# benoriol/hand_pose_sl

Hardware: NVIDIA B200
Metric: body2hand_train_frames_per_sec (higher is better)
Workload: dtype bf16

## Files before the change

hand_pose_sl_b200/csrc/b2h_capi.cu:

```cuda
#include <atomic>
#include <cstdarg>
#include <cstdio>
#include <mutex>
#include <cmath>

#include "b2h_common.cuh"

namespace b2h {

static thread_local char g_err[512] = "";
static std::atomic<long long> g_launches{0};

void set_error(const char* fmt, ...) {
  va_list ap;
  va_start(ap, fmt);
  vsnprintf(g_err, sizeof(g_err), fmt, ap);
  va_end(ap);
}
int check_launch(const char* what) {
  cudaError_t e = cudaGetLastError();
  if (e != cudaSuccess) {
    set_error("%s: %s", what, cudaGetErrorString(e));
    return B2H_ECUDA;
  }
// ... 231 lines not shown
  if ((reinterpret_cast<uintptr_t>(x) & 15) || (reinterpret_cast<uintptr_t>(target) & talign) ||
      (reinterpret_cast<uintptr_t>(conf) & calign) || (reinterpret_cast<uintptr_t>(packed) & 15)) {
    if (wv) set_error("%s: frames and packed must be 16-byte aligned, target_frames 8-byte and conf_frames 4-byte aligned", who);
    else set_error("%s: x, target and packed must be 16-byte aligned", who);
    return B2H_EALIGN;
  }
  g = make_geo(n_in, C, pos_emb);
  plan = train_plan(g, B, T, precision);
  if (wv && plan.kernel != B2H_KERNEL_TC_TILE && plan.kernel != B2H_KERNEL_TC_WIDE_TRAIN) {
    set_error("%s: window views are trained on the tensor cores: in bf16 mode for conv_channels <= 32 with at most 32 input "
              "channels and T <= 4096, and for conv_channels <= 256 with T <= 256; in fp32 mode for conv_channels <= 32 with at "
              "most 32 input channels and T <= 4096; materialise the windows (b2h_preprocess) for C=%d, T=%d, precision=%d",
              who, C, T, precision);
    return B2H_ESHAPE;
  }
  if (plan.kernel == B2H_KERNEL_NONE) {
    set_error("%s: no training kernel for conv_channels=%d, T=%d, precision=%d (tcgen05 training: C <= 32 in the one-launch tile "
              "kernel, C <= 256 in bf16 mode through the wide kernels, T <= 256; the FFMA kernel would need %zu B of shared memory)",
              who, C, T, precision, plan.ffma.smem);
    return B2H_ESHAPE;
  }
  const int nparts = plan.nparts;
  const int64_t stride = plan.stride;
  if (workspace_bytes < plan.total - 256) { set_error("%s: workspace %lld B < %lld B", who, (long long)workspace_bytes, (long long)plan.total); return B2H_EWORKSPACE; }
  if (reinterpret_cast<uintptr_t>(workspace) & 15) { set_error("%s: workspace must be 16-byte aligned", who); return B2H_EALIGN; }
  partials = reinterpret_cast<float*>(reinterpret_cast<char*>(workspace) + B2H_WS_HEADER);
  loss_partials = partials + (size_t)nparts * stride;
  Fp32Args a{};
  a.x = x; a.x_dtype = x_dtype; a.target = target; a.conf = conf; a.d_y = d_y; a.lengths = lengths; a.params = params;
  a.packed = reinterpret_cast<const char*>(packed); a.y = pred_out; a.partials = partials; a.loss_partials = loss_partials;
  a.B = B; a.T = T; a.loss_kind = loss_kind; a.apply_mask = 1; a.mode = mode; a.out_scale = 1.0f; a.geo = g;
  a.step_dev = step_dev;
  a.epoch_dev = epoch_dev;
  if (wv) a.wv = *wv;
  if (plan.kernel == B2H_KERNEL_TC_TILE) {
    if (fuse) {
      if (nparts > B2H_WS_MAX_CTA) { set_error("%s: %d CTAs exceed the %d arrival flags of the workspace header", who, nparts, B2H_WS_MAX_CTA); return B2H_ESHAPE; }
      fuse->enabled = 1;
      fuse->hdr = reinterpret_cast<unsigned*>(workspace);
      a.fuse = *fuse;
    }
    return launch_tc_tile_train(a, plan.tile, stream);
  }
  if (plan.kernel == B2H_KERNEL_TC_WIDE_TRAIN) {
    return launch_tc_wide_train(a, plan.wide, reinterpret_cast<unsigned char*>(workspace) + plan.scratch_off, stream);
  }
  return launch_fp32(a, plan.ffma, stream);
}

static int train_forward_backward(const void* x, int x_dtype, const WindowView* wv, const float* target, const float* conf,
                                  const int32_t* lengths, const float* params, const void* packed, float* grads_out,
                                  float* loss_out, float* pred_out, int B, int T, int n_in, int C, int pos_emb, int loss_kind,
                                  int precision, int64_t* step_dev, void* workspace, int64_t workspace_bytes, void* stream,
                                  const char* who) {
  if (grads_out && !loss_out) { set_error("%s: null loss_out", who); return B2H_EINVAL; }
  Geo g; TrainPlan plan; float *partials, *loss_partials;
  int rc = train_common(x, x_dtype, wv, target, conf, nullptr, lengths, params, packed, pred_out, B, T, n_in, C, pos_emb,
                        loss_kind, precision, 1, workspace, workspace_bytes, (cudaStream_t)stream, g, plan, partials,
                        loss_partials, who, reinterpret_cast<long long*>(step_dev));
  if (rc || !grads_out) return rc;
  return launch_reduce(partials, plan.nparts, plan.gp_layout, g, grads_out, loss_partials, loss_out, (cudaStream_t)stream, nullptr, plan.n_loss);
}

extern "C" int b2h_train_forward_backward(const void* x, int x_dtype, const float* target, const float* conf,
                                          const int32_t* lengths, const float* params, const void* packed,
                                          float* grads_out, float* loss_out, float* pred_out, int B, int T, int n_in,
// ... 228 lines not shown
```

hand_pose_sl_b200/csrc/b2h_common.cuh:

```cuda
#pragma once
#include <cuda_runtime.h>
#include <cuda_bf16.h>
#include <stdint.h>
#include "../../include/b2h.h"

#define B2H_KW 5
#define B2H_PADW 2
#define B2H_COUT 42
#define B2H_MAX_C 256

namespace b2h {

__host__ __device__ inline int round_up(int x, int m) { return (x + m - 1) / m * m; }

struct Geo {
  int n_in, C, pos_emb;
  int pe_len;
  int cin[4], cout[4];
  int w_off[4], b_off[4];
  int P;
  int64_t wf_off[4];
  int64_t wd_off[4];
  int64_t tf_off[4];
  int64_t td_off[4];
// ... 125 lines not shown
  const float denom = sqrtf(v) * inv_bc2_sqrt + eps;
  return p - step_size * (m / denom);
}

__host__ __device__ inline double ipow(double b, long long t) {
  double r = 1.0;
  while (t > 0) {
    if (t & 1) r *= b;
    b *= b;
    t >>= 1;
  }
  return r;
}

struct SubWindow { int start, clo, chi; };
__host__ __device__ inline int sub_window_cut(int T, int Ts, int n_sub, int i) {
  if (i <= 0) return 0;
  if (i >= n_sub) return T;
  const int c = (Ts - 16) + (i - 1) * (Ts - 32);
  return c < T ? c : T;
}
__host__ __device__ inline SubWindow sub_window(int T, int Ts, int n_sub, int i) {
  SubWindow s;
  const int cb0 = sub_window_cut(T, Ts, n_sub, i), cb1 = sub_window_cut(T, Ts, n_sub, i + 1);
  int st = cb0 - 16;
  st = st < 0 ? 0 : st;
  st = st > T - Ts ? T - Ts : st;
  s.start = st; s.clo = cb0 - st; s.chi = cb1 - st;
  return s;
}

#define B2H_WS_HEADER 1024
#define B2H_WS_MAX_CTA 192

struct FuseAdam {
  int enabled;
  float* params; float* m; float* v; char* packed;
  double lr, beta1, beta2;
  const double* lr_dev;
  float eps, grad_scale;
  const long long* step_dev;
  float* loss_out;
  unsigned* hdr;
  const float* const* peer_bufs;
  float* sym_grads;
  unsigned long long* mc_buf;
  const long long* epoch_dev;
  int rank, world;
};

void set_error(const char* fmt, ...);
int check_launch(const char* what);
void count_launch(int n = 1);


struct WindowView { const long long* win_start; const long long* win_end; long long n_frames; int pad_mode; };

__device__ __forceinline__ long long window_src_row(const WindowView& v, int w, int t) {
  const long long start = v.win_start[w];
  long long cend = v.win_end ? v.win_end[w] : v.n_frames;
  cend = cend > v.n_frames ? v.n_frames : cend;
  long long f = start + t;
  if (f >= cend || f < 0) f = (v.pad_mode == B2H_PAD_REPEAT_FIRST && start >= 0 && start < cend) ? start : -1;
  return f;
}

// ... 14 lines not shown
  size_t smem;
  int grid;
};
RowspacePlan plan_rowspace(const Geo& g, int B, int T);

struct WidePlan {
  bool ok;
  int gh, n_tiles, a_bytes, nstage;
  size_t smem;
  int grid;
  int ksplit;
  int n_loss;
  int64_t scratch_bytes;
};
WidePlan plan_wide(const Geo& g, int B, int T);

struct FfmaPlan {
  bool ok, train;
  size_t smem;
  int grid;
};
FfmaPlan plan_ffma(const Geo& g, int B, int T, bool train);

struct Fp32Args {
  const void* x; int x_dtype;
  const float* target; const float* conf; const float* d_y; const int32_t* lengths;
  const float* params; const char* packed;
  float* y;
  float* partials;
  float* loss_partials;
  long long* step_dev;
  long long* epoch_dev;
  FuseAdam fuse;
  int B, T, loss_kind, apply_mask, mode;
  float out_scale;
  Geo geo;
  WindowView wv;
};
int launch_fp32(Fp32Args& p, const FfmaPlan& plan, cudaStream_t stream);

struct TcFwdArgs {
  const void* x; int x_dtype;
  const float* params; const char* packed; const int32_t* lengths;
  float* y;
  int B, T, G, NT, RBUF, apply_mask;
  float out_scale;
  Geo geo;
  WindowView wv;
};
int launch_tc_fwd(TcFwdArgs& p, const RowspacePlan& plan, cudaStream_t stream);
int launch_tc_wide_train(const Fp32Args& a, const WidePlan& plan, unsigned char* scratch, cudaStream_t stream);
int launch_tc_wide_fwd(const void* x, int x_dtype, const float* params, const char* packed, const int32_t* lengths, float* y,
                       int B, int T, int apply_mask, float out_scale, const Geo& g, const WidePlan& plan, cudaStream_t stream,
                       const WindowView* wv);
int launch_tc_probe(const void* a, const void* b, float* out, int n, int ksteps, int shift, int variant, cudaStream_t stream);
int tc_status_and_clear();

int launch_tc_tile_fwd(const void* x, int x_dtype, const float* params, const char* packed, const int32_t* lengths, float* y,
                       int apply_mask, float out_scale, const Geo& g, const TilePlan& plan, cudaStream_t stream, const WindowView* wv);
int launch_tc_tile_train(const Fp32Args& a, const TilePlan& plan, cudaStream_t stream);

void set_debug_timing(long long* p);
int launch_tc_bench(long long* out, int M, int N, int reps, int nacc, int mn_major, cudaStream_t stream);
int launch_format_prediction(const float* pred, float* out, int64_t rows, int mode, cudaStream_t stream);
int launch_pos_emb_concat(const float* inp, float* out, int B, int Cc, int T, int max_len, cudaStream_t stream);
int launch_pack(const float* params, void* packed, const Geo& g, cudaStream_t stream);
// ... 17 lines not shown
```

hand_pose_sl_b200/csrc/b2h_conv_fp32.cu:

```cuda
#include "b2h_common.cuh"

namespace b2h {

constexpr int kThreads = 256;
constexpr int kWarps = kThreads / 32;



template <int EPI>
__device__ __forceinline__ void conv_rows(const float* __restrict__ in, int ldi, int Cin, const float* __restrict__ W,
                                          int Cout, const float* __restrict__ bias, float* __restrict__ out, int ldo,
                                          const float* __restrict__ act, int lda, int T) {
  const int lane = threadIdx.x & 31, warp = threadIdx.x >> 5;
  const int nRB = (T + 7) >> 3, nCG = (Cout + 31) >> 5;
  for (int task = warp; task < nRB * nCG; task += kWarps) {
    const int rb = task / nCG, cg = task - rb * nCG;
    const int co = cg * 32 + lane;
    const bool active = co < Cout;
    const int r0 = rb * 8;
    float acc[8];
    const float b0 = (EPI != 2 && active) ? __ldg(bias + co) : 0.0f;
#pragma unroll
    for (int j = 0; j < 8; ++j) acc[j] = b0;
    const float* xin = in + r0 * ldi;
// ... 75 lines not shown
  for (int w = 0; w < kWarps; ++w) s += red[w];
  return s;
}

template <bool TRAIN>
__global__ void __launch_bounds__(kThreads) conv_fp32_kernel(Fp32Args p) {
  extern __shared__ __align__(16) float smem[];
  __shared__ float red[kWarps];
  const Geo& g = p.geo;
  const int T = p.T;
  const int TR = round_up(T, 8) + 4;
  const int ld0 = round_up(g.cin[0], 4), ldc = round_up(g.C, 4), ldg = round_up(g.C > B2H_COUT ? g.C : B2H_COUT, 4);
  float* X = smem;
  float* A1 = X + TR * ld0;
  float* A2 = A1 + TR * ldc;
  float* A3 = A2 + TR * ldc;
  float* G0 = A3 + TR * ldc;
  float* G1 = G0 + TR * ldg;
  const int total = TRAIN ? TR * (ld0 + 3 * ldc + 2 * ldg) : TR * (ld0 + 2 * ldc);
  for (int i = threadIdx.x; i < total; i += kThreads) smem[i] = 0.0f;
  __syncthreads();

  const float* Wf[4];
  const float* Wd[4];
  const float* bias[4];
#pragma unroll
  for (int l = 0; l < 4; ++l) {
    Wf[l] = reinterpret_cast<const float*>(p.packed + g.wf_off[l]);
    Wd[l] = reinterpret_cast<const float*>(p.packed + g.wd_off[l]);
    bias[l] = p.params + g.b_off[l];
  }
  if (TRAIN && p.step_dev && blockIdx.x == 0 && threadIdx.x == 0) *p.step_dev += 1;
  if (TRAIN && p.epoch_dev && blockIdx.x == 0 && threadIdx.x == 0) *p.epoch_dev += 1;
  float* part = TRAIN ? p.partials + (size_t)blockIdx.x * g.P : nullptr;
  float loss_acc = 0.0f;
  bool first = true;

  for (int b = blockIdx.x; b < p.B; b += gridDim.x) {
    const int n_in = g.n_in, pe = g.pos_emb;
    if (p.x_dtype == B2H_DT_F32) {
      const float* xs = reinterpret_cast<const float*>(p.x) + (size_t)b * T * n_in;
      for (int i = threadIdx.x; i < T * n_in; i += kThreads) {
        int t = i / n_in, c = i - t * n_in;
        X[(t + 2) * ld0 + pe + c] = __ldg(xs + i);
      }
    } else {
      const __nv_bfloat16* xs = reinterpret_cast<const __nv_bfloat16*>(p.x) + (size_t)b * T * n_in;
      for (int i = threadIdx.x; i < T * n_in; i += kThreads) {
        int t = i / n_in, c = i - t * n_in;
        X[(t + 2) * ld0 + pe + c] = __bfloat162float(xs[i]);
      }
    }
    if (pe) {
      for (int t = threadIdx.x; t < T; t += kThreads) X[(t + 2) * ld0] = __fdiv_rn((float)t, (float)g.pe_len);
    }
    __syncthreads();
    conv_rows<0>(X, ld0, g.cin[0], Wf[0], g.cout[0], bias[0], A1, ldc, nullptr, 0, T);
    __syncthreads();
    conv_rows<0>(A1, ldc, g.cin[1], Wf[1], g.cout[1], bias[1], A2, ldc, nullptr, 0, T);
    __syncthreads();
    int len = T;
    if (p.lengths) { len = p.lengths[b]; len = len < 0 ? 0 : (len > T ? T : len); }

    if (!TRAIN) {
      conv_rows<0>(A2, ldc, g.cin[2], Wf[2], g.cout[2], bias[2], A1, ldc, nullptr, 0, T);
      __syncthreads();
// ... 138 lines not shown
```

hand_pose_sl_b200/csrc/b2h_train_tc.cuh:

```cuda
#pragma once
#include <type_traits>

namespace b2h {
using namespace tc;

struct TcTileArgs {
  const void* x; int x_dtype;
  const float* target; const float* conf; const float* d_y; const int32_t* lengths;
  const float* params; const char* packed;
  float* y;
  float* partials;
  float* loss_partials;
  long long* step_dev;
  long long* epoch_dev;
  long long* dbg;
  FuseAdam fuse;
  const long long* win_start; const long long* win_end; long long n_frames; int pad_mode;
  int T_orig, n_sub, loss_B;
  int B, T, loss_kind, apply_mask, mode;
  float out_scale;
  int n_tiles, nhalf, MB, HR, gh, NT;
  Geo geo;
};

constexpr int kTileThreads = 256;
constexpr int kAccCol = 0;
constexpr int kWgPairCols = 5 * 32 + 8;
constexpr int kGatherDepth = 24;
constexpr uint32_t kDpSentinel = 0xFFFFFFFFu;

struct TileSmem {
  int g0, g1, x, a1, a2, a3, ones, lo_off, ys, has_ys, wf[4], wlo_off, wd[4], total;
};

__host__ __device__ inline TileSmem tile_smem_layout(const Geo& g, int rows, bool train, bool split = false) {
  TileSmem s;
  const int CH = rows * 16;
  int o = 0;
  s.g0 = o; o += train ? 6 * CH : 0;
  s.g1 = o; o += train ? 4 * CH : 0;
  s.x = o;  o += (g.kp[0] / 8) * CH;
  s.a1 = o; o += (g.kp[1] / 8) * CH;
  s.a2 = o; o += (g.kp[1] / 8) * CH;
  s.a3 = o; o += train ? (g.kp[1] / 8) * CH : 0;
  s.ones = o; o += train ? CH : 0;
  s.lo_off = split ? o : 0;
  if (split) o *= 2;
// ... 57 lines not shown
      const uint32_t a = a_lo + 2 * s * rows + k, b = b_lo + (k * KS + s) * 2 * N;
      umma_bf16(d_tmem, desc64(a, a_hi), desc64(b, b_hi), idesc, acc);
      acc = 1;
      if (SPLIT) {
        umma_bf16(d_tmem, desc64(a + al16, a_hi), desc64(b, b_hi), idesc, 1);
        umma_bf16(d_tmem, desc64(a, a_hi), desc64(b + bl16, b_hi), idesc, 1);
      }
    }
  }
}

__device__ __forceinline__ void grid_barrier_flags(unsigned* hdr, unsigned tok, int tid) {
  __syncthreads();
  volatile unsigned* flags = hdr + 4;
  if (tid == 0) {
    __threadfence();
    flags[blockIdx.x] = tok;
  }
  if (tid < 32) {
    const long long t0 = clock64();
    for (;;) {
      bool mine = true;
      for (int c = tid; c < (int)gridDim.x; c += 32) mine = mine && (flags[c] == tok);
      if (__all_sync(0xffffffffu, mine)) break;
      if (clock64() - t0 > 4000000000LL) {
        if (tid == 0) atomicExch(&g_tc_status, 50);
        break;
      }
    }
    __threadfence();
  }
  __syncthreads();
}

__device__ __forceinline__ void adam_apply(const FuseAdam& f, const Geo& g, const GpSlot& slot, int i, float gr, float m, float v,
                                           float p, float step_size, float inv_bc2_sqrt) {
  p = adam_update(m, v, p, gr * f.grad_scale, (float)(1.0 - f.beta1), (float)(1.0 - f.beta2), (float)f.beta2, f.eps, step_size,
                  inv_bc2_sqrt);
  f.m[i] = m; f.v[i] = v; f.params[i] = p;
  if (f.packed) scatter_packed(g, f.packed, slot, p);
}

#define B2H_STAMP() do { if (p.dbg && blockIdx.x == 0 && tid == 0 && dbg_n < 120) p.dbg[dbg_n++] = clock64(); } while (0)
__device__ __forceinline__ long long global_ns() { long long t; asm volatile("mov.u64 %0, %globaltimer;" : "=l"(t)); return t; }
#define B2H_MARK(i) do { if (p.dbg && tid == 0 && blockIdx.x < 192) p.dbg[128 + 4 * blockIdx.x + (i)] = global_ns(); } while (0)

template <bool TRAIN, int NT, bool SPLIT, bool VIEW = false>
__global__ void __launch_bounds__(kTileThreads, 1) conv_tc_tile_kernel(TcTileArgs p) {
  int dbg_n = 0;
  extern __shared__ __align__(128) unsigned char smem[];
  __shared__ __align__(8) uint64_t bar;
  __shared__ __align__(8) uint64_t wbar;
  __shared__ __align__(8) uint64_t tbar;
  __shared__ uint32_t tmem_slot;
  __shared__ __align__(16) float bias_s[4][64];
  __shared__ float red_s[8];
  const Geo& g = p.geo;
  const int T = p.T, MB = p.MB, HR = p.HR, nhalf = p.nhalf, gh = p.gh;
  constexpr int kWgCol = 64 * NT;
  const int tid = threadIdx.x, lane = tid & 31;
  const int warp = __shfl_sync(0xffffffffu, tid >> 5, 0);
  const int rows = nhalf * HR;
  const int CH = rows * 16;
  const TileSmem L = tile_smem_layout(g, rows, TRAIN, SPLIT);
  const int LO = L.lo_off;
  const uint32_t al16 = (uint32_t)L.lo_off >> 4, bl16 = (uint32_t)L.wlo_off >> 4;
// ... 97 lines not shown
    mbar_init(&bar, nissue);
    mbar_init(&wbar, 1);
    mbar_init(&tbar, 1);
    fence_barrier_init();
  }
  auto zero_buffers = [&]() {
    const int act_bytes = L.ys;
    uint4* z = reinterpret_cast<uint4*>(smem);
    const uint4 zero = make_uint4(0, 0, 0, 0);
    for (int i = tid; i < act_bytes / 16; i += kTileThreads) z[i] = zero;
  };
  if (!TRAIN) zero_buffers();
  griddep_wait();
  B2H_STAMP();
  prefetch_x(blockIdx.x);
  if (tid == 0) {
    uint32_t total = 4 * 64 * 4;
    for (int l = 0; l < 4; ++l) {
      total += B2H_KW * g.kp[l] * g.np_[l] * 2 * (SPLIT ? 2 : 1);
      if (TRAIN && !SPLIT && l > 0) total += B2H_KW * round_up(g.cout[l], 16) * round_up(g.cin[l], 16) * 2;
    }
    mbar_arrive_expect_tx(&wbar, total);
    bulk_g2s(&bias_s[0][0], p.packed + g.bias_off, 4 * 64 * 4, &wbar);
    for (int l = 0; l < 4; ++l) {
      bulk_g2s(smem + L.wf[l], p.packed + g.tf_off[l], B2H_KW * g.kp[l] * g.np_[l] * 2, &wbar);
      if (SPLIT) bulk_g2s(smem + L.wf[l] + L.wlo_off, p.packed + g.tfl_off[l], B2H_KW * g.kp[l] * g.np_[l] * 2, &wbar);
      if (TRAIN && !SPLIT && l > 0)
        bulk_g2s(smem + L.wd[l], p.packed + g.td_off[l], B2H_KW * round_up(g.cout[l], 16) * round_up(g.cin[l], 16) * 2, &wbar);
    }
  }
  long long step_next = 0, epoch_next = 0;
  unsigned sync_tok = 0;
  int abort_flag = 0;
  if (TRAIN) {
    if (p.fuse.enabled) {
      step_next = *reinterpret_cast<const volatile long long*>(p.fuse.step_dev) + 1;
      if (p.fuse.world > 1) {
        epoch_next = *reinterpret_cast<const volatile long long*>(p.fuse.epoch_dev) + 1;
        abort_flag = *reinterpret_cast<volatile int*>(&g_dp_abort);
      }
      sync_tok = *reinterpret_cast<const volatile unsigned*>(p.fuse.hdr) + 1u;
    } else if (blockIdx.x == 0 && tid == 0) {
      if (p.step_dev) *p.step_dev += 1;
      if (p.epoch_dev) *p.epoch_dev += 1;
    }
  }
  if (TRAIN) zero_buffers();
  tc_fence_before();
  __syncthreads();
  tc_fence_after();
  const uint32_t tbase = tmem_slot;
  uint32_t phase = 0, tphase = 0;
  float loss_acc = 0.0f;
  bool wg_started = false, weights_ready = false;
  B2H_STAMP();

  const uint32_t hi_k = desc_hi(128);
  const uint32_t hi_mn = desc_hi((uint32_t)CH);
  const uint32_t acc_d = tbase + kAccCol;

  bool pair1_done = false;
  auto readout_pair = [&](int pr) {
    float* part = p.partials + (size_t)blockIdx.x * gp_total(g);
    const int l = 2 * pr + (lane >> 4);
    const int co = (warp & 3) * 16 + (lane & 15);
    const bool mine = co < g.cout[l];
    const int Nw = g.kp[l];
    float* lp = part + gp_layer_off(g, l);
    float4* lp4 = reinterpret_cast<float4*>(lp);
    const int q4 = Nw >> 2, cout_l = g.cout[l];
    const uint32_t dcol = tbase + lane_addr + kWgCol + pr * kWgPairCols;
    const int k0 = ch == 0 ? 0 : 3, nk = ch == 0 ? 3 : 2;
    uint32_t v[3][32];
#pragma unroll
    for (int k = 0; k < 3; ++k)
      if (k < nk) tmem_ld32(dcol + (k0 + k) * 32, v[k]);
    uint32_t vb[16];
    if (ch == 1) tmem_ld16(dcol + 5 * 32, vb);
    tmem_ld_wait();
    if (mine) {
#pragma unroll
      for (int k = 0; k < 3; ++k) {
        if (k >= nk) continue;
        float4* dst = lp4 + (size_t)(k0 + k) * q4 * cout_l + co;
#pragma unroll
        for (int q = 0; q < 8; ++q)
          if (q * 4 < Nw)
            dst[(size_t)q * cout_l] = make_float4(__uint_as_float(v[k][4 * q]), __uint_as_float(v[k][4 * q + 1]),
                                                  __uint_as_float(v[k][4 * q + 2]), __uint_as_float(v[k][4 * q + 3]));
      }
      if (ch == 1) lp[B2H_KW * g.cout[l] * Nw + co] = __uint_as_float(vb[0]);
    }
  };

  for (int tile = blockIdx.x; tile < p.n_tiles; tile += gridDim.x) {
    const int wbase = tile * wpt;
    int lens[NT];
#pragma unroll
    for (int j = 0; j < NT; ++j) {
      const RowCtx rc = rowctx(j, wbase);
      const int Tw = p.n_sub > 1 ? p.T_orig : T;
      lens[j] = Tw;
      if (rc.valid && p.lengths) { const int v = p.lengths[p.n_sub > 1 ? rc.gw / p.n_sub : rc.gw]; lens[j] = v < 0 ? 0 : (v > Tw ? Tw : v); }
    }

    const bool tgt_smem = TRAIN && p.mode == 1 && bulk_io && p.n_sub <= 1;
    if (tid == 0) {
      if (!TRAIN) bulk_wait_read0();
      if (tgt_smem) {
        int nw = p.B - wbase; nw = nw > wpt ? wpt : nw;
        fence_proxy_async_smem();
        if (!VIEW) {
          mbar_arrive_expect_tx(&tbar, (uint32_t)nw * T * B2H_COUT * 4);
          for (int w = 0; w < nw; ++w) {
            const int h = w / gh, j = w - h * gh;
            bulk_g2s(YS + (size_t)(h * MB + j * (T + 2)) * B2H_COUT, p.target + (size_t)(wbase + w) * T * B2H_COUT,
                     (uint32_t)T * B2H_COUT * 4, &tbar);
          }
        } else {
          int nb = 0;
          for (int w = 0; w < nw; ++w) nb += view_bulk(wbase + w) ? 1 : 0;
          mbar_arrive_expect_tx(&tbar, (uint32_t)nb * T * B2H_COUT * 4);
          for (int w = 0; w < nw; ++w) {
            if (!view_bulk(wbase + w)) continue;
            const int h = w / gh, j = w - h * gh;
// ... 57 lines not shown
        float2* dst = reinterpret_cast<float2*>(YS + (size_t)srow * B2H_COUT);
        for (int q = ch * 11; q < (ch ? B2H_COUT / 2 : 11); ++q) dst[q] = tr < 0 ? make_float2(0.f, 0.f) : __ldg(src + q);
      }
      if (TRAIN && ch == 0) {
        uint4 o = make_uint4(0, 0, 0, 0);
        if (rc.valid) o.x = 0x00003F80u;
        *reinterpret_cast<uint4*>(ONES + (size_t)row * 16) = o;
      }
    }
    prefetch_x(tile + gridDim.x);
    fence_proxy_async_smem();
    tc_fence_before();
    __syncthreads();
    tc_fence_after();
    B2H_STAMP();
    if (!weights_ready) { mbar_wait(&wbar, 0, 19); weights_ready = true; }
    B2H_STAMP();

    for (int l = 0; l < 4; ++l) {
      unsigned char* bin = (l == 0) ? X : (l == 1) ? A1 : (l == 2) ? A2 : (TRAIN ? A3 : A1);
      unsigned char* bout = (l == 0) ? A1 : (l == 1) ? A2 : (TRAIN ? A3 : A1);
      const int KS = g.kp[l] >> 4, N = g.np_[l];
      if (warp < nissue) {
        if (elect_one()) {
          const uint32_t idesc = make_idesc_bf16(idesc_M, N, 0, 0);
          const uint32_t a_lo = desc_lo(smem_u32(bin), (uint32_t)CH) + warp * seg_row;
          const uint32_t b_lo = desc_lo(smem_u32(smem + L.wf[l]), (uint32_t)N * 16);
          issue_conv<SPLIT>(acc_d + warp * seg_d, a_lo, hi_k, b_lo, hi_k, KS, N, rows, idesc, al16, bl16);
          umma_commit(&bar);
        }
        __syncwarp();
      }
      B2H_STAMP();
      mbar_wait(&bar, phase, 20 + l);
      phase ^= 1;
      tc_fence_after();
      B2H_STAMP();
      float contrib = 0.f;
#pragma unroll
      for (int j = 0; j < NT; ++j) {
      const RowCtx rc = rowctx(j, wbase);
      const int row = rc.row, t = rc.t, gw = rc.gw;
      const bool valid = rc.valid;
      const uint32_t taddr = tbase + lane_addr + kAccCol + 64 * j;
      if (l < 3) {
        for (int c0 = 16 * ch; c0 < N; c0 += 32) {
          uint32_t v[16];
          tmem_ld16(taddr + c0, v);
          tmem_ld_wait();
          float f[16];
#pragma unroll
          for (int q = 0; q < 16; ++q) f[q] = valid ? fmaxf(__uint_as_float(v[q]) + bias_s[l][c0 + q], 0.0f) : 0.0f;
          store8_act<SPLIT>(bout, LO, CH, row, c0 >> 3, f);
          store8_act<SPLIT>(bout, LO, CH, row, (c0 >> 3) + 1, f + 8);
        }
      } else {
        int len = lens[j];
        float n_el = 0.f, scale = 0.f;
        const float* tg = nullptr; const float* cf = nullptr; const float* dy = nullptr;
        const size_t drow = valid ? (size_t)dense_row(gw, t) : 0;
        bool in_core = true, zrow = false;
        if (TRAIN && valid) {
          n_el = (float)len * (float)B2H_COUT;
          scale = (p.loss_kind == B2H_LOSS_L1) ? (1.0f / (float)p.loss_B) / n_el : 1.0f / n_el;
          if (p.n_sub > 1) {
            const SubW sw = subw(gw);
// ... 212 lines not shown
          const int row = rc.row;
          const bool valid = rc.valid;
          const uint32_t taddr = tbase + lane_addr + kAccCol + 64 * j;
          for (int c0 = 16 * ch; c0 < Nd; c0 += 32) {
            uint32_t v[16];
            tmem_ld16(taddr + c0, v);
            tmem_ld_wait();
            float f[16], act[16];
            bf16x8_to_float(*reinterpret_cast<const uint4*>(ain + (size_t)(c0 >> 3) * CH + (size_t)row * 16), act);
            bf16x8_to_float(*reinterpret_cast<const uint4*>(ain + (size_t)((c0 >> 3) + 1) * CH + (size_t)row * 16), act + 8);
#pragma unroll
            for (int q = 0; q < 16; ++q) f[q] = (valid && act[q] > 0.0f) ? __uint_as_float(v[q]) : 0.0f;
            store8_act<SPLIT>(gnext, LO, CH, row, c0 >> 3, f);
            store8_act<SPLIT>(gnext, LO, CH, row, (c0 >> 3) + 1, f + 8);
          }
          }
        }
        if (l == 1 && tile + (int)gridDim.x >= p.n_tiles) {
          readout_pair(1);
          pair1_done = true;
        }
        fence_proxy_async_smem();
        tc_fence_before();
        __syncthreads();
        tc_fence_after();
        B2H_STAMP();
      }
      wg_started = true;
    }
  }

  if (TRAIN) {
    if (!wg_started) {
      float* part = p.partials + (size_t)blockIdx.x * gp_total(g);
      for (int i = tid; i < gp_total(g); i += kTileThreads) part[i] = 0.0f;
    } else {
      readout_pair(0);
      if (!pair1_done) readout_pair(1);
    }
    if (tid == 0 && p.loss_partials)
      p.loss_partials[blockIdx.x] = (p.loss_kind == B2H_LOSS_L1) ? loss_acc / (float)p.loss_B : loss_acc;
    B2H_STAMP();

    if (p.fuse.enabled) {
      const FuseAdam& f = p.fuse;
      __shared__ float s_step_size, s_inv_bc2_sqrt;
      const int nj = gp_total(g);
      const int nparts = (int)gridDim.x;
      const int per = round_up((nj + nparts - 1) / nparts, 4);
      const int j0 = (int)blockIdx.x * per;
      const int j_end = min(nj, j0 + per);
      const bool dp = f.world > 1;
      if (tid == kTileThreads - 1) {
        const float lr = (float)(f.lr_dev ? *f.lr_dev : f.lr);
        const float tt = (float)step_next;
        const float bc1 = -expm1f(tt * log1pf((float)(f.beta1 - 1.0)));
        const float bc2 = -expm1f(tt * log1pf((float)(f.beta2 - 1.0)));
        s_step_size = lr / bc1;
        s_inv_bc2_sqrt = 1.0f / sqrtf(bc2);
      }
      const bool one_pass = per <= kTileThreads;
      GpSlot my_slot;
      int my_i = -1;
      float my_m = 0.f, my_v = 0.f, my_p = 0.f;
      if (one_pass && j0 + tid < j_end && gp_decode(g, j0 + tid, my_slot)) {
        my_i = gp_flat_of_slot(g, my_slot);
        my_m = __ldcg(f.m + my_i); my_v = __ldcg(f.v + my_i); my_p = __ldcg(f.params + my_i);
      }
      B2H_MARK(1);
      bool aborted = abort_flag != 0;
      grid_barrier_flags(f.hdr, sync_tok, tid);
      B2H_STAMP();
      B2H_MARK(2);
      if (blockIdx.x == 0 && tid == 0) {
        *reinterpret_cast<volatile unsigned*>(f.hdr) = sync_tok;
        *p.step_dev = step_next;
        if (dp) *p.epoch_dev = epoch_next;
      }
      if (blockIdx.x == 0 && warp == 7 && f.loss_out) {
        float sl = 0.f;
        for (int c = lane; c < (int)gridDim.x; c += 32) sl += __ldcg(p.loss_partials + c);
#pragma unroll
        for (int o = 16; o > 0; o >>= 1) sl += __shfl_xor_sync(0xffffffffu, sl, o);
        if (lane == 0) *f.loss_out = sl;
      }
      const long long epoch = epoch_next;
      const size_t ll_src = ((size_t)(epoch & 1) * f.world + f.rank) * nj;
      float4* red4 = reinterpret_cast<float4*>(L.has_ys ? smem + L.ys : smem);
      for (int jb = j0; jb < j_end; jb += 4096) {
        const int jn = min(j_end, jb + 4096);
        const int ncol = (jn - jb + 3) >> 2;
        int groups = kTileThreads / ncol; groups = groups < 1 ? 1 : (groups > 8 ? 8 : groups);
        const int cpg = kTileThreads / groups;
        for (int cb = 0; cb < ncol; cb += cpg) {
          const int col = cb + tid % cpg, pg = tid / cpg;
          if (col < ncol && pg < groups) {
            const float4* src = reinterpret_cast<const float4*>(p.partials + jb + 4 * col);
            const size_t stride4 = (size_t)nj >> 2;
            float4 acc = make_float4(0.f, 0.f, 0.f, 0.f);
            for (int c = pg; c < nparts; c += kGatherDepth * groups) {
              float4 v[kGatherDepth];
#pragma unroll
              for (int u = 0; u < kGatherDepth; ++u) {
                const int cc = c + u * groups;
                v[u] = (cc < nparts) ? __ldcg(src + (size_t)cc * stride4) : make_float4(0.f, 0.f, 0.f, 0.f);
              }
#pragma unroll
              for (int u = 0; u < kGatherDepth; ++u) { acc.x += v[u].x; acc.y += v[u].y; acc.z += v[u].z; acc.w += v[u].w; }
            }
            red4[pg * ncol + col] = acc;
          }
        }
        __syncthreads();
        B2H_STAMP();
        const float* red = reinterpret_cast<const float*>(red4);
        for (int j = jb + tid; j < jn; j += kTileThreads) {
          float gr = 0.f;
          for (int pg = 0; pg < groups; ++pg) gr += red[(size_t)pg * ncol * 4 + (j - jb)];
          bool apply = true;
          const bool real_slot = one_pass ? (my_i >= 0) : (flat_index_of_gp(g, j) >= 0);
          if (dp && real_slot) {
            uint32_t word = __float_as_uint(gr);
            if (word == kDpSentinel) word = 0x7FC00000u;
            if (f.mc_buf) {
              asm volatile("multimem.st.relaxed.sys.global.b32 [%0], %1;" ::"l"(reinterpret_cast<uint32_t*>(f.mc_buf) + ll_src + j), "r"(word) : "memory");
            } else {
              for (int r = 0; r < f.world; ++r)
                *(reinterpret_cast<volatile uint32_t*>(const_cast<float*>(f.peer_bufs[r])) + ll_src + j) = word;
            }
            B2H_STAMP();
            float gsum = 0.f;
            volatile uint32_t* mine = reinterpret_cast<volatile uint32_t*>(const_cast<float*>(f.peer_bufs[f.rank])) + (size_t)(epoch & 1) * f.world * nj + j;
            const long long t0 = clock64();
            for (int rb = 0; rb < f.world; rb += 8) {
              uint32_t w[8];
              bool all_here;
              do {
#pragma unroll
                for (int u = 0; u < 8; ++u)
                  if (rb + u < f.world) w[u] = mine[(size_t)(rb + u) * nj];
                all_here = true;
#pragma unroll
                for (int u = 0; u < 8; ++u)
                  if (rb + u < f.world) all_here = all_here && (w[u] != kDpSentinel);
                if (!all_here && clock64() - t0 > 6000000000LL) {
                  atomicExch(&g_tc_status, 51);
                  atomicExch(&g_dp_abort, 1);
                  aborted = true;
                  break;
                }
              } while (!all_here);
#pragma unroll
              for (int u = 0; u < 8; ++u)
                if (rb + u < f.world) {
                  gsum += __uint_as_float(w[u]);
                  if (!aborted) mine[(size_t)(rb + u) * nj] = kDpSentinel;
                }
            }
            B2H_STAMP();
            gr = gsum;
            apply = !aborted;
          }
          if (apply) {
            if (one_pass) {
              if (my_i >= 0) adam_apply(f, g, my_slot, my_i, gr, my_m, my_v, my_p, s_step_size, s_inv_bc2_sqrt);
            } else {
              GpSlot sl;
              if (gp_decode(g, j, sl)) {
                const int i = gp_flat_of_slot(g, sl);
                adam_apply(f, g, sl, i, gr, f.m[i], f.v[i], f.params[i], s_step_size, s_inv_bc2_sqrt);
              }
            }
          }
        }
        __syncthreads();
      }
      B2H_STAMP();
      B2H_MARK(3);
    }
  }
  if (!TRAIN && tid == 0) bulk_wait0();
  B2H_STAMP();
  tc_fence_before();
  __syncthreads();
  if (warp == 0) tmem_dealloc(tbase, TRAIN ? 512 : 64 * NT);
}

constexpr int kTileMaxTrainT = 4096;

TilePlan plan_tile(const Geo& g, int B, int T, bool train, bool split) {
  TilePlan p{};
  p.train = train; p.split = split;
  if (T < 1 || T > (train ? kTileMaxTrainT : 256)) return p;
  if ((g.kp[0] > 32 || g.kp[1] > 32) && (train || split || g.kp[0] > 64 || g.kp[1] > 64)) return p;
  p.n_sub = 1;
  const int Ts = split ? 128 : 256;
  if (train && T > Ts) {
    p.n_sub = 2;
    while (2 * (Ts - 16) + (p.n_sub - 2) * (Ts - 32) < T) ++p.n_sub;
  }
  p.B = B * p.n_sub;
  p.T = p.n_sub > 1 ? Ts : T;
  if (p.T <= 64) { p.nhalf = 2; p.MB = 64; p.NT = 1; }
  else { p.nhalf = 1; p.NT = (p.T > 128) ? 2 : 1; p.MB = 128 * p.NT; }
  p.HR = p.MB + 8;
  p.gh = (p.MB + 2) / (p.T + 2);
  const int wpt = p.nhalf * p.gh;
  p.n_tiles = (p.B + wpt - 1) / wpt;
// ... 37 lines not shown
    at[0].id = cudaLaunchAttributeProgrammaticStreamSerialization;
    at[0].val.programmaticStreamSerializationAllowed = 1;
    at[1].id = cudaLaunchAttributeCooperative;
    at[1].val.cooperative = 1;
    cfg.attrs = at; cfg.numAttrs = coop ? 2 : 1;
    le = cudaLaunchKernelExC(&cfg, fn, kargs);
  } else if (coop) {
    le = cudaLaunchCooperativeKernel(fn, dim3(grid), dim3(kTileThreads), kargs, smem, stream);
  } else {
    le = cudaLaunchKernel(fn, dim3(grid), dim3(kTileThreads), kargs, smem, stream);
  }
  if (le != cudaSuccess) { cudaGetLastError(); set_error("tile kernel launch: %s", cudaGetErrorString(le)); return B2H_ECUDA; }
  count_launch();
  return check_launch(train ? "conv_tc_tile_kernel<train>" : "conv_tc_tile_kernel<fwd>");
}

static long long* g_dbg_timing = nullptr;
void set_debug_timing(long long* p) { g_dbg_timing = p; }

int launch_tc_tile_fwd(const void* x, int x_dtype, const float* params, const char* packed, const int32_t* lengths, float* y,
                       int apply_mask, float out_scale, const Geo& g, const TilePlan& plan, cudaStream_t stream, const WindowView* wv) {
  TcTileArgs p{};
  p.x = x; p.x_dtype = x_dtype; p.params = params; p.packed = packed; p.lengths = lengths; p.y = y;
  p.apply_mask = apply_mask; p.mode = 0; p.out_scale = out_scale; p.geo = g;
  if (wv) { p.win_start = wv->win_start; p.win_end = wv->win_end; p.n_frames = wv->n_frames; p.pad_mode = wv->pad_mode; }
  p.dbg = g_dbg_timing;
  return launch_tc_tile(p, plan, stream);
}

int launch_tc_tile_train(const Fp32Args& a, const TilePlan& plan, cudaStream_t stream) {
  TcTileArgs p{};
  p.x = a.x; p.x_dtype = a.x_dtype; p.target = a.target; p.conf = a.conf; p.d_y = a.d_y; p.lengths = a.lengths;
  p.params = a.params; p.packed = a.packed; p.y = a.y; p.partials = a.partials; p.loss_partials = a.loss_partials;
  p.step_dev = a.step_dev; p.epoch_dev = a.epoch_dev; p.loss_kind = a.loss_kind; p.apply_mask = 1; p.mode = a.mode;
  p.out_scale = 1.0f; p.geo = a.geo;
  p.fuse = a.fuse;
  p.dbg = g_dbg_timing;
  p.loss_B = a.B; p.T_orig = a.T; p.n_sub = plan.n_sub;
  p.win_start = a.wv.win_start; p.win_end = a.wv.win_end; p.n_frames = a.wv.n_frames; p.pad_mode = a.wv.pad_mode;
  return launch_tc_tile(p, plan, stream);
}

}
```

hand_pose_sl_b200/csrc/b2h_wide_tc.cuh:

```cuda
#pragma once
#include <cuda.h>

namespace b2h {
using namespace tc;

struct WideStageDesc { int KS, N, row0, layer; };

struct WideArgs {
  const void* x; int x_dtype;
  const float* params; const char* packed; const int32_t* lengths;
  float* y;
  long long* dbg;
  int B, T, apply_mask;
  float out_scale;
  int n_tiles, gh, nstage, a_bytes;
  Geo geo;
  int n_stages;
  WideStageDesc st[4];
  const float* target; const float* conf; const float* d_y;
  int loss_kind, train_mode;
  unsigned char* scratch;
  long long tile_bytes;
  long long act_off[4], dz_off[4];
  float* loss_partials;
  long long* step_dev; long long* epoch_dev;
  WindowView wv;
};

constexpr int kWideThreads = 320;
constexpr int kWideEpiThreads = 256;
constexpr int kWideRows = 264;
constexpr int kWideStage = 16384;
constexpr int kWideBoxRows = kWideStage / 128;
constexpr int kWideMaxStages = 16;

struct WideSched { int KS, N, blk_bytes, nblk, bps, nst; };
__host__ __device__ inline WideSched wide_sched(int KS, int N) {
  WideSched s;
  s.KS = KS; s.N = N;
  s.blk_bytes = s.N * 32;
  s.nblk = B2H_KW * s.KS;
  s.bps = kWideStage / s.blk_bytes; if (s.bps < 1) s.bps = 1;
  s.nst = (s.nblk + s.bps - 1) / s.bps;
  return s;
}

struct WideScratch { long long act_off[4], dz_off[4], tile_bytes; };
__host__ __device__ inline WideScratch wide_scratch(const Geo& g) {
  WideScratch w;
  long long o = 0;
  const long long CHB = (long long)kWideRows * 16;
  for (int l = 0; l < 4; ++l) { w.act_off[l] = o; o += (g.kp[l] / 8) * CHB; }
  for (int l = 0; l < 4; ++l) { w.dz_off[l] = o; o += (g.np_[l] / 8) * CHB; }
  w.tile_bytes = o;
  return w;
}

// ... 31 lines not shown
  __shared__ __align__(8) uint64_t act_ready;
  __shared__ uint32_t tmem_slot;
  __shared__ __align__(16) float bias_s[4][256];
  __shared__ float loss_w[8];
  const Geo& g = p.geo;
  const int T = p.T, gh = p.gh;
  const int tid = threadIdx.x, lane = tid & 31;
  const int warp = __shfl_sync(0xffffffffu, tid >> 5, 0);
  constexpr int rows = kWideRows;
  constexpr int CH = rows * 16;
  unsigned char* A = smem;
  unsigned char* RING = smem + p.a_bytes;
  const int S = p.nstage;
  const int NL = p.n_stages;

  for (int i = tid; i < 4 * 256; i += kWideThreads) {
    const int l = i >> 8, c = i & 255;
    bias_s[l][c] = c < g.cout[l] ? __ldg(p.params + g.b_off[l] + c) : 0.0f;
  }
  {
    uint4* z = reinterpret_cast<uint4*>(A);
    const uint4 zero = make_uint4(0, 0, 0, 0);
    for (int i = tid; i < p.a_bytes / 16; i += kWideThreads) z[i] = zero;
  }
  if (warp == 0) tmem_alloc(&tmem_slot, 512);
  if (tid == 0) {
    for (int s = 0; s < S; ++s) { mbar_init(&full_bar[s], 1); mbar_init(&empty_bar[s], 1); }
    mbar_init(&acc_full, 1);
    mbar_init(&act_ready, kWideEpiThreads);
    fence_barrier_init();
    if (MODE == 1 && blockIdx.x == 0) {
      if (p.step_dev) *p.step_dev += 1;
      if (p.epoch_dev) *p.epoch_dev += 1;
    }
  }
  fence_proxy_async_smem();
  tc_fence_before();
  __syncthreads();
  tc_fence_after();
  const uint32_t tbase = tmem_slot;

  const uint32_t full0 = smem_u32(&full_bar[0]), empty0 = smem_u32(&empty_bar[0]), ring0 = smem_u32(RING);
  if (warp == 9) {
    if (elect_one()) {
      uint32_t slot = 0, ph = 1;
      for (int tile = blockIdx.x; tile < p.n_tiles; tile += gridDim.x)
        for (int l = 0; l < NL; ++l) {
          const WideSched sc = wide_sched(p.st[l].KS, p.st[l].N);
          int row = p.st[l].row0;
          const int rows_per_stage = (sc.bps * sc.blk_bytes) >> 7;
          for (int st = 0; st < sc.nst; ++st) {
            if (!wait_addr(empty0 + slot * 8, ph, 60)) return;
            expect_tx_addr(full0 + slot * 8, kWideStage);
            tma_load_2d_addr(ring0 + slot * kWideStage, &wmap, 0, row, full0 + slot * 8);
            row += rows_per_stage;
            if (++slot == (uint32_t)S) { slot = 0; ph ^= 1; }
          }
        }
    }
    __syncwarp();
  } else if (warp == 8) {
    if (elect_one()) {
      uint32_t slot = 0, ph = 0, act_phase = 0;
      int dn = 0;
      const uint32_t hi_k = desc_hi(128);
      const uint32_t a_lo0 = desc_lo(smem_u32(A), (uint32_t)CH);
// ... 551 lines not shown
  for (int l = 0; l < 4; ++l) { p.act_off[l] = ws.act_off[l]; p.dz_off[l] = ws.dz_off[l]; }
}

static void wide_forward_stages(WideArgs& p, const Geo& g) {
  p.n_stages = 4;
  for (int l = 0; l < 4; ++l) { p.st[l].KS = g.kp[l] >> 4; p.st[l].N = g.np_[l]; p.st[l].row0 = (int)((g.tf_off[l] - g.tf_off[0]) >> 7); p.st[l].layer = l; }
}

int launch_tc_wide_fwd(const void* x, int x_dtype, const float* params, const char* packed, const int32_t* lengths, float* y,
                       int B, int T, int apply_mask, float out_scale, const Geo& g, const WidePlan& plan, cudaStream_t stream,
                       const WindowView* wv) {
  WideArgs p{};
  p.x = x; p.x_dtype = x_dtype; p.params = params; p.packed = packed; p.lengths = lengths; p.y = y;
  p.apply_mask = apply_mask; p.out_scale = out_scale;
  if (wv) p.wv = *wv;
  wide_common(p, g, plan, B, T);
  wide_forward_stages(p, g);
  if (int rc = ensure_dyn_smem(reinterpret_cast<const void*>(conv_tc_wide_kernel<0>), plan.smem)) return rc;
  CUtensorMap wmap;
  if (int rc = wide_weight_map(packed + g.tf_off[0], g.td_off[0] - g.tf_off[0], &wmap)) return rc;
  conv_tc_wide_kernel<0><<<plan.grid, kWideThreads, plan.smem, stream>>>(p, wmap);
  count_launch();
  return check_launch("conv_tc_wide_kernel<fwd>");
}

int launch_tc_wide_train(const Fp32Args& a, const WidePlan& plan, unsigned char* scratch, cudaStream_t stream) {
  const Geo& g = a.geo;
  WideArgs p{};
  p.x = a.x; p.x_dtype = a.x_dtype; p.params = a.params; p.packed = a.packed; p.lengths = a.lengths; p.y = a.y;
  p.apply_mask = 1; p.out_scale = 1.0f;
  p.target = a.target; p.conf = a.conf; p.d_y = a.d_y; p.loss_kind = a.loss_kind; p.train_mode = a.mode;
  p.scratch = scratch; p.loss_partials = a.loss_partials;
  p.step_dev = a.step_dev; p.epoch_dev = a.epoch_dev;
  p.wv = a.wv;
  wide_common(p, g, plan, a.B, a.T);
  const size_t smem = plan.smem;
  const int grid = plan.grid;
  wide_forward_stages(p, g);
  auto* fwd = p.wv.win_start ? conv_tc_wide_kernel<1, true> : conv_tc_wide_kernel<1>;
  if (int rc = ensure_dyn_smem(reinterpret_cast<const void*>(fwd), smem)) return rc;
  CUtensorMap fmap, bmap;
  if (int rc = wide_weight_map(a.packed + g.tf_off[0], g.td_off[0] - g.tf_off[0], &fmap)) return rc;
  fwd<<<grid, kWideThreads, smem, stream>>>(p, fmap);
  count_launch();
  if (int rc = check_launch("conv_tc_wide_kernel<train fwd>")) return rc;
  if (int rc = wide_weight_map(a.packed + g.td_off[1], g.tfl_off[0] - g.td_off[1], &bmap)) return rc;
  p.n_stages = 3;
  for (int j = 0; j < 3; ++j) {
    const int l = 3 - j;
    p.st[j].KS = g.np_[l] >> 4; p.st[j].N = g.kp[l]; p.st[j].row0 = (int)((g.td_off[l] - g.td_off[1]) >> 7); p.st[j].layer = l;
  }
  if (int rc = ensure_dyn_smem(reinterpret_cast<const void*>(conv_tc_wide_kernel<2>), smem)) return rc;
  conv_tc_wide_kernel<2><<<grid, kWideThreads, smem, stream>>>(p, bmap);
  count_launch();
  if (int rc = check_launch("conv_tc_wide_kernel<dgrad>")) return rc;
  WgradArgs w{};
  w.scratch = scratch; w.tile_bytes = p.tile_bytes;
  for (int l = 0; l < 4; ++l) { w.act_off[l] = p.act_off[l]; w.dz_off[l] = p.dz_off[l]; }
  w.n_tiles = p.n_tiles; w.partials = a.partials; w.geo = g;
  w.n_items = wide_wgrad_items(g, w.items);
  if (w.n_items <= 0) { set_error("wide wgrad: too many work items"); return B2H_ESHAPE; }
  w.ksplit = plan.ksplit;
  const size_t wsmem = (size_t)2 * kWgStageBytes + 2 * kWgChunkB;
  if (int rc = ensure_dyn_smem(reinterpret_cast<const void*>(conv_tc_wide_wgrad_kernel), wsmem)) return rc;
  CUtensorMap smap;
  if (int rc = wide_weight_map(reinterpret_cast<const char*>(scratch), (int64_t)p.n_tiles * p.tile_bytes, &smap, kWgBoxRows)) return rc;
// ... 7 lines not shown
```

Measured before the change: 586.1 million.

## Replace fused-Adam grid barrier with sentinel-based per-slice readiness polling

In the fused one-launch training kernel, the full grid barrier before gradient reduction is skipped when the workspace header is 'armed' from the previous step. Consumers instead poll each partial slice for a sentinel value, with relaxed loads and a timeout, and reset slices to the sentinel after reading them. Producers write partials with relaxed stores that scrub any accidental sentinel values, and non-fused kernels disarm the header. This removes the global barrier wait so reduction can start as soon as each slice lands, at the cost of extra polling, extra sentinel writes, and tricky memory-ordering correctness.

```diff
diff --git a/hand_pose_sl_b200/csrc/b2h_capi.cu b/hand_pose_sl_b200/csrc/b2h_capi.cu
--- a/hand_pose_sl_b200/csrc/b2h_capi.cu
+++ b/hand_pose_sl_b200/csrc/b2h_capi.cu
@@ -287,6 +287,7 @@
   a.B = B; a.T = T; a.loss_kind = loss_kind; a.apply_mask = 1; a.mode = mode; a.out_scale = 1.0f; a.geo = g;
   a.step_dev = step_dev;
   a.epoch_dev = epoch_dev;
+  a.ws_hdr = reinterpret_cast<unsigned*>(workspace);
   if (wv) a.wv = *wv;
   if (plan.kernel == B2H_KERNEL_TC_TILE) {
     if (fuse) {
diff --git a/hand_pose_sl_b200/csrc/b2h_common.cuh b/hand_pose_sl_b200/csrc/b2h_common.cuh
--- a/hand_pose_sl_b200/csrc/b2h_common.cuh
+++ b/hand_pose_sl_b200/csrc/b2h_common.cuh
@@ -181,6 +181,7 @@
 
 #define B2H_WS_HEADER 1024
 #define B2H_WS_MAX_CTA 192
+#define B2H_WS_ARMED (4 + B2H_WS_MAX_CTA)
 
 struct FuseAdam {
   int enabled;
@@ -261,6 +262,7 @@
   long long* step_dev;
   long long* epoch_dev;
   FuseAdam fuse;
+  unsigned* ws_hdr;
   int B, T, loss_kind, apply_mask, mode;
   float out_scale;
   Geo geo;
diff --git a/hand_pose_sl_b200/csrc/b2h_conv_fp32.cu b/hand_pose_sl_b200/csrc/b2h_conv_fp32.cu
--- a/hand_pose_sl_b200/csrc/b2h_conv_fp32.cu
+++ b/hand_pose_sl_b200/csrc/b2h_conv_fp32.cu
@@ -131,6 +131,7 @@
   }
   if (TRAIN && p.step_dev && blockIdx.x == 0 && threadIdx.x == 0) *p.step_dev += 1;
   if (TRAIN && p.epoch_dev && blockIdx.x == 0 && threadIdx.x == 0) *p.epoch_dev += 1;
+  if (TRAIN && p.ws_hdr && blockIdx.x == 0 && threadIdx.x == 0) p.ws_hdr[B2H_WS_ARMED] = 0u;
   float* part = TRAIN ? p.partials + (size_t)blockIdx.x * g.P : nullptr;
   float loss_acc = 0.0f;
   bool first = true;
diff --git a/hand_pose_sl_b200/csrc/b2h_train_tc.cuh b/hand_pose_sl_b200/csrc/b2h_train_tc.cuh
--- a/hand_pose_sl_b200/csrc/b2h_train_tc.cuh
+++ b/hand_pose_sl_b200/csrc/b2h_train_tc.cuh
@@ -13,6 +13,7 @@
   float* loss_partials;
   long long* step_dev;
   long long* epoch_dev;
+  unsigned* ws_hdr;
   long long* dbg;
   FuseAdam fuse;
   const long long* win_start; const long long* win_end; long long n_frames; int pad_mode;
@@ -136,6 +137,31 @@
   }
   __syncthreads();
 }
+
+__device__ __forceinline__ uint32_t scrub_sentinel(float v) { const uint32_t w = __float_as_uint(v); return w == kDpSentinel ? 0x7FC00000u : w; }
+__device__ __forceinline__ void st_slice4(float* p, float a, float b, float c, float d) {
+  asm volatile("st.relaxed.gpu.global.v4.b32 [%0], {%1, %2, %3, %4};" ::"l"(p), "r"(scrub_sentinel(a)), "r"(scrub_sentinel(b)),
+               "r"(scrub_sentinel(c)), "r"(scrub_sentinel(d)) : "memory");
+}
+__device__ __forceinline__ void st_slice1(float* p, float a) {
+  asm volatile("st.relaxed.gpu.global.b32 [%0], %1;" ::"l"(p), "r"(scrub_sentinel(a)) : "memory");
+}
+__device__ __forceinline__ float4 ld_slice4(const float* p) {
+  uint32_t a, b, c, d;
+  asm volatile("ld.relaxed.gpu.global.v4.b32 {%0, %1, %2, %3}, [%4];" : "=r"(a), "=r"(b), "=r"(c), "=r"(d) : "l"(p) : "memory");
+  return make_float4(__uint_as_float(a), __uint_as_float(b), __uint_as_float(c), __uint_as_float(d));
+}
+__device__ __forceinline__ float ld_slice1(const float* p) {
+  uint32_t a;
+  asm volatile("ld.relaxed.gpu.global.b32 %0, [%1];" : "=r"(a) : "l"(p) : "memory");
+  return __uint_as_float(a);
+}
+__device__ __forceinline__ bool slice4_missing(const float4& v) {
+  return (__float_as_uint(v.x) == kDpSentinel) | (__float_as_uint(v.y) == kDpSentinel) | (__float_as_uint(v.z) == kDpSentinel) |
+         (__float_as_uint(v.w) == kDpSentinel);
+}
+__device__ __forceinline__ void fence_acq_rel_gpu() { asm volatile("fence.acq_rel.gpu;" ::: "memory"); }
+constexpr long long kSliceWaitCycles = 4000000000LL;
 
 __device__ __forceinline__ void adam_apply(const FuseAdam& f, const Geo& g, const GpSlot& slot, int i, float gr, float m, float v,
                                            float p, float step_size, float inv_bc2_sqrt) {
@@ -299,6 +325,7 @@
   long long step_next = 0, epoch_next = 0;
   unsigned sync_tok = 0;
   int abort_flag = 0;
+  __shared__ __align__(16) unsigned s_rec[4];
   if (TRAIN) {
     if (p.fuse.enabled) {
       step_next = *reinterpret_cast<const volatile long long*>(p.fuse.step_dev) + 1;
@@ -307,9 +334,12 @@
         abort_flag = *reinterpret_cast<volatile int*>(&g_dp_abort);
       }
       sync_tok = *reinterpret_cast<const volatile unsigned*>(p.fuse.hdr) + 1u;
+      if (tid == 0)
+        asm volatile("cp.async.cg.shared.global [%0], [%1], 16;" ::"r"(smem_u32(s_rec)), "l"(p.fuse.hdr + B2H_WS_ARMED) : "memory");
     } else if (blockIdx.x == 0 && tid == 0) {
       if (p.step_dev) *p.step_dev += 1;
       if (p.epoch_dev) *p.epoch_dev += 1;
+      if (p.ws_hdr) p.ws_hdr[B2H_WS_ARMED] = 0u;
     }
   }
   if (TRAIN) zero_buffers();
@@ -353,11 +383,11 @@
 #pragma unroll
         for (int q = 0; q < 8; ++q)
           if (q * 4 < Nw)
-            dst[(size_t)q * cout_l] = make_float4(__uint_as_float(v[k][4 * q]), __uint_as_float(v[k][4 * q + 1]),
-                                                  __uint_as_float(v[k][4 * q + 2]), __uint_as_float(v[k][4 * q + 3]));
-      }
-      if (ch == 1) lp[B2H_KW * g.cout[l] * Nw + co] = __uint_as_float(vb[0]);
-    }
+            st_slice4(reinterpret_cast<float*>(dst + (size_t)q * cout_l), __uint_as_float(v[k][4 * q]), __uint_as_float(v[k][4 * q + 1]),
+                      __uint_as_float(v[k][4 * q + 2]), __uint_as_float(v[k][4 * q + 3]));
+      }
+    }
+    if (ch == 1 && co < round_up(cout_l, 4)) st_slice1(lp + B2H_KW * cout_l * Nw + co, mine ? __uint_as_float(vb[0]) : 0.0f);
   };
 
   for (int tile = blockIdx.x; tile < p.n_tiles; tile += gridDim.x) {
@@ -481,6 +511,10 @@
         __syncwarp();
       }
       B2H_STAMP();
+      if (TRAIN && p.fuse.enabled && l == 0 && tile == (int)blockIdx.x) {
+        if (tid == 0) asm volatile("cp.async.wait_all;" ::: "memory");
+        fence_acq_rel_gpu();
+      }
       mbar_wait(&bar, phase, 20 + l);
       phase ^= 1;
       tc_fence_after();
@@ -759,14 +793,18 @@
 
   if (TRAIN) {
     if (!wg_started) {
+      if (p.fuse.enabled) {
+        if (tid == 0) asm volatile("cp.async.wait_all;" ::: "memory");
+        fence_acq_rel_gpu();
+      }
       float* part = p.partials + (size_t)blockIdx.x * gp_total(g);
-      for (int i = tid; i < gp_total(g); i += kTileThreads) part[i] = 0.0f;
+      for (int i = tid; i < gp_total(g) / 4; i += kTileThreads) st_slice4(part + 4 * i, 0.0f, 0.0f, 0.0f, 0.0f);
     } else {
       readout_pair(0);
       if (!pair1_done) readout_pair(1);
     }
     if (tid == 0 && p.loss_partials)
-      p.loss_partials[blockIdx.x] = (p.loss_kind == B2H_LOSS_L1) ? loss_acc / (float)p.loss_B : loss_acc;
+      st_slice1(p.loss_partials + blockIdx.x, (p.loss_kind == B2H_LOSS_L1) ? loss_acc / (float)p.loss_B : loss_acc);
     B2H_STAMP();
 
     if (p.fuse.enabled) {
@@ -796,24 +834,33 @@
       }
       B2H_MARK(1);
       bool aborted = abort_flag != 0;
-      grid_barrier_flags(f.hdr, sync_tok, tid);
+      if (tid == 0) asm volatile("cp.async.wait_all;" ::: "memory");
+      __syncthreads();
+      const bool armed = s_rec[0] == sync_tok && s_rec[1] == gridDim.x && s_rec[2] == (unsigned)nj;
+      if (!armed) grid_barrier_flags(f.hdr, sync_tok, tid);
       B2H_STAMP();
-      B2H_MARK(2);
-      if (blockIdx.x == 0 && tid == 0) {
-        *reinterpret_cast<volatile unsigned*>(f.hdr) = sync_tok;
-        *p.step_dev = step_next;
-        if (dp) *p.epoch_dev = epoch_next;
-      }
-      if (blockIdx.x == 0 && warp == 7 && f.loss_out) {
-        float sl = 0.f;
-        for (int c = lane; c < (int)gridDim.x; c += 32) sl += __ldcg(p.loss_partials + c);
-#pragma unroll
-        for (int o = 16; o > 0; o >>= 1) sl += __shfl_xor_sync(0xffffffffu, sl, o);
-        if (lane == 0) *f.loss_out = sl;
+      if (blockIdx.x == 0 && warp == 7) {
+        float ls = 0.f;
+        const long long t0 = clock64();
+        for (int c = lane; c < nparts; c += 32) {
+          float* w = p.loss_partials + c;
+          float v = ld_slice1(w);
+          while (__float_as_uint(v) == kDpSentinel) {
+            if (clock64() - t0 > kSliceWaitCycles) { atomicExch(&g_tc_status, 50); break; }
+            __nanosleep(64);
+            v = ld_slice1(w);
+          }
+          *w = __uint_as_float(kDpSentinel);
+          ls += v;
+        }
+#pragma unroll
+        for (int o = 16; o > 0; o >>= 1) ls += __shfl_xor_sync(0xffffffffu, ls, o);
+        if (lane == 0 && f.loss_out) *f.loss_out = ls;
       }
       const long long epoch = epoch_next;
       const size_t ll_src = ((size_t)(epoch & 1) * f.world + f.rank) * nj;
       float4* red4 = reinterpret_cast<float4*>(L.has_ys ? smem + L.ys : smem);
+      B2H_MARK(2);
       for (int jb = j0; jb < j_end; jb += 4096) {
         const int jn = min(j_end, jb + 4096);
         const int ncol = (jn - jb + 3) >> 2;
@@ -822,22 +869,54 @@
         for (int cb = 0; cb < ncol; cb += cpg) {
           const int col = cb + tid % cpg, pg = tid / cpg;
           if (col < ncol && pg < groups) {
-            const float4* src = reinterpret_cast<const float4*>(p.partials + jb + 4 * col);
-            const size_t stride4 = (size_t)nj >> 2;
+            float* src = p.partials + jb + 4 * col;
             float4 acc = make_float4(0.f, 0.f, 0.f, 0.f);
             for (int c = pg; c < nparts; c += kGatherDepth * groups) {
               float4 v[kGatherDepth];
 #pragma unroll
               for (int u = 0; u < kGatherDepth; ++u) {
                 const int cc = c + u * groups;
-                v[u] = (cc < nparts) ? __ldcg(src + (size_t)cc * stride4) : make_float4(0.f, 0.f, 0.f, 0.f);
+                v[u] = (cc < nparts) ? ld_slice4(src + (size_t)cc * nj) : make_float4(0.f, 0.f, 0.f, 0.f);
               }
+              uint32_t miss = 0;
+#pragma unroll
+              for (int u = 0; u < kGatherDepth; ++u) miss |= slice4_missing(v[u]) ? 1u << u : 0u;
+              if (miss) {
+                const long long t0 = clock64();
+                unsigned ns = 32;
+                do {
+                  __nanosleep(ns);
+                  ns = ns < 256 ? 2 * ns : 256;
+                  const int first = __ffs(miss) - 1;
+                  bool landed = false;
+#pragma unroll
+                  for (int u = 0; u < kGatherDepth; ++u)
+                    if (u == first) { v[u] = ld_slice4(src + (size_t)(c + u * groups) * nj); landed = !slice4_missing(v[u]); }
+                  if (!landed) {
+                    if (clock64() - t0 > kSliceWaitCycles) { atomicExch(&g_tc_status, 50); break; }
+                    continue;
+                  }
+#pragma unroll
+                  for (int u = 0; u < kGatherDepth; ++u)
+                    if (u != first && ((miss >> u) & 1u)) v[u] = ld_slice4(src + (size_t)(c + u * groups) * nj);
+                  miss = 0;
+#pragma unroll
+                  for (int u = 0; u < kGatherDepth; ++u) miss |= slice4_missing(v[u]) ? 1u << u : 0u;
+                  if (miss && clock64() - t0 > kSliceWaitCycles) { atomicExch(&g_tc_status, 50); break; }
+                } while (miss);
+              }
+              const float sent = __uint_as_float(kDpSentinel);
+#pragma unroll
+              for (int u = 0; u < kGatherDepth; ++u)
+                if (c + u * groups < nparts) *reinterpret_cast<float4*>(src + (size_t)(c + u * groups) * nj) = make_float4(sent, sent, sent, sent);
 #pragma unroll
               for (int u = 0; u < kGatherDepth; ++u) { acc.x += v[u].x; acc.y += v[u].y; acc.z += v[u].z; acc.w += v[u].w; }
             }
             red4[pg * ncol + col] = acc;
           }
         }
+        if (p.dbg && jb == j0 && blockIdx.x < 192) atomicMax(reinterpret_cast<unsigned long long*>(p.dbg + 128 + 4 * blockIdx.x + 2), (unsigned long long)global_ns());
+        fence_acq_rel_gpu();
         __syncthreads();
         B2H_STAMP();
         const float* red = reinterpret_cast<const float*>(red4);
@@ -901,6 +980,15 @@
           }
         }
         __syncthreads();
+      }
+      if (blockIdx.x == 0 && tid == 0) {
+        volatile unsigned* h = f.hdr;
+        h[0] = sync_tok;
+        h[B2H_WS_ARMED] = sync_tok + 1u;
+        h[B2H_WS_ARMED + 1] = gridDim.x;
+        h[B2H_WS_ARMED + 2] = (unsigned)nj;
+        *p.step_dev = step_next;
+        if (dp) *p.epoch_dev = epoch_next;
       }
       B2H_STAMP();
       B2H_MARK(3);
@@ -1004,7 +1092,7 @@
   TcTileArgs p{};
   p.x = a.x; p.x_dtype = a.x_dtype; p.target = a.target; p.conf = a.conf; p.d_y = a.d_y; p.lengths = a.lengths;
   p.params = a.params; p.packed = a.packed; p.y = a.y; p.partials = a.partials; p.loss_partials = a.loss_partials;
-  p.step_dev = a.step_dev; p.epoch_dev = a.epoch_dev; p.loss_kind = a.loss_kind; p.apply_mask = 1; p.mode = a.mode;
+  p.step_dev = a.step_dev; p.epoch_dev = a.epoch_dev; p.ws_hdr = a.ws_hdr; p.loss_kind = a.loss_kind; p.apply_mask = 1; p.mode = a.mode;
   p.out_scale = 1.0f; p.geo = a.geo;
   p.fuse = a.fuse;
   p.dbg = g_dbg_timing;
diff --git a/hand_pose_sl_b200/csrc/b2h_wide_tc.cuh b/hand_pose_sl_b200/csrc/b2h_wide_tc.cuh
--- a/hand_pose_sl_b200/csrc/b2h_wide_tc.cuh
+++ b/hand_pose_sl_b200/csrc/b2h_wide_tc.cuh
@@ -23,6 +23,7 @@
   long long tile_bytes;
   long long act_off[4], dz_off[4];
   float* loss_partials;
+  unsigned* ws_hdr;
   long long* step_dev; long long* epoch_dev;
   WindowView wv;
 };
@@ -120,6 +121,7 @@
     if (MODE == 1 && blockIdx.x == 0) {
       if (p.step_dev) *p.step_dev += 1;
       if (p.epoch_dev) *p.epoch_dev += 1;
+      if (p.ws_hdr) p.ws_hdr[B2H_WS_ARMED] = 0u;
     }
   }
   fence_proxy_async_smem();
@@ -737,6 +739,7 @@
   p.target = a.target; p.conf = a.conf; p.d_y = a.d_y; p.loss_kind = a.loss_kind; p.train_mode = a.mode;
   p.scratch = scratch; p.loss_partials = a.loss_partials;
   p.step_dev = a.step_dev; p.epoch_dev = a.epoch_dev;
+  p.ws_hdr = a.ws_hdr;
   p.wv = a.wv;
   wide_common(p, g, plan, a.B, a.T);
   const size_t smem = plan.smem;
```

After: 564.4 million (median of 6 runs). 3.7% lower.
